# deargen/DeepInteract

Measured on AMD Instinct MI355X. Metric: complexes/sec GeoT+pair-tensor fwd (2×1k res, k=20, 1/8 GPU); % HBM peak, higher is better.
Workload: dtype bf16

## Files before the change

__graft_entry__.py:

```python
import os
import sys

ROOT = os.path.dirname(os.path.abspath(__file__))
if ROOT not in sys.path:
    sys.path.insert(0, ROOT)


def build() -> None:
    from deepinteract_amd import build as _b
    _b.build(force=False)
    import deepinteract_amd
    from deepinteract_amd import _lib
    _lib.load(build_if_missing=False)
    from deepinteract_amd.build import build_variant
    from tools.build_variants import VARIANTS
    for name in ("node2", "f32exact"):
        try:
            build_variant(name, VARIANTS[name])
        except RuntimeError as e:
            print(f"variant {name} failed to build (test_gpu_variants will fail):\n{e}", file=sys.stderr)


def smoke() -> None:
    import numpy as np
    import torch

    from deepinteract_amd.engine import GeoTEngine, PairTensorOp
    from deepinteract_amd.graph import GraphBatch
    from deepinteract_amd.weights import seeded_state_dict
    from oracle import geot_oracle as O

    z = np.load(os.path.join(ROOT, "tests", "golden", "tiny.npz"))
    items, graphs = [], []
    for tag in ("g1", "g2"):
        it = {"num_nodes": int(z[f"{tag}_node_f"].shape[0])}
        for k in ("src", "dst", "src_nbr", "dst_nbr"):
            it[k] = torch.as_tensor(z[f"{tag}_{k}"]).long()
        it["node_f"] = torch.as_tensor(z[f"{tag}_node_f"])
        it["edge_f"] = torch.as_tensor(z[f"{tag}_edge_f"])
        items.append(it)
    sd = seeded_state_dict(0, with_head=False)
    eng = GeoTEngine(sd, "f32", device="cuda:0")
    gb = GraphBatch.from_arrays(items, "cuda:0")
    h, e = eng.forward(gb)
    n1 = items[0]["num_nodes"]
    _, views = PairTensorOp("cuda:0")(h, [0], [n1], [n1], [items[1]["num_nodes"]])
    torch.cuda.synchronize()
    with torch.no_grad():
        ref = [O.geot_forward(sd, it) for it in items]
    ref_h = torch.cat([r[0] for r in ref]).numpy()
    got = h.cpu().numpy()
    err = np.abs(got - ref_h).max() / np.abs(ref_h).max()
    pt_ref = O.pair_tensor(torch.as_tensor(ref_h[:n1]), torch.as_tensor(ref_h[n1:])).numpy()
    perr = np.abs(views[0].cpu().numpy() - pt_ref).max() / np.abs(pt_ref).max()
    print(f"smoke: GeoT node rel err {err:.2e}, pair tensor rel err {perr:.2e}")
    if not (err < 1e-4 and perr < 1e-4):
        raise AssertionError(f"smoke parity failed: {err}, {perr}")


if __name__ == "__main__":
    build()
    if len(sys.argv) > 1 and sys.argv[1] == "smoke":
        smoke()
```

deepinteract_amd/csrc/common.h:

```cpp
#pragma once
#include <hip/hip_runtime.h>
#include <stdint.h>

#include <atomic>

namespace di {

inline int device_cus() {
  constexpr int MAXDEV = 64;
  static std::atomic<int> cache[MAXDEV];
  int dev = 0;
  if (hipGetDevice(&dev) != hipSuccess || dev < 0) dev = 0;
  if (dev < MAXDEV) {
    const int c = cache[dev].load(std::memory_order_relaxed);
    if (c > 0) return c;
  }
  int v = 0;
  if (hipDeviceGetAttribute(&v, hipDeviceAttributeMultiprocessorCount, dev) != hipSuccess || v <= 0) v = 256;
  if (dev < MAXDEV) cache[dev].store(v, std::memory_order_relaxed);
  return v;
}

typedef float floatx4 __attribute__((ext_vector_type(4)));
typedef float floatx2 __attribute__((ext_vector_type(2)));
// ... 287 lines not shown
    const int bo = blk(i), s = kst(i);
    out.v[bo] = __builtin_amdgcn_mfma_f32_16x16x32_bf16(fr[i % D], op.f[s], out.v[bo], 0, 0, 0);
    if (i + D < N)
      fr[i % D] = *reinterpret_cast<const bf16x8*>(w + (blk(i + D) * NS + kst(i + D)) * BLK + lane * 8);
  }
  __builtin_amdgcn_sched_barrier(0);
}

template <int NBO, int NS>
__device__ __forceinline__ void mma(Act<NBO>& out, const Op<BF16T, NS>& op, const u16* w, int lane) {
  constexpr int G = NBO < 2 ? NBO : 2;
#pragma unroll
  for (int b0 = 0; b0 < NBO; b0 += G) {
#pragma unroll
    for (int s = 0; s < NS; ++s) {
#pragma unroll
      for (int bo = b0; bo < b0 + G; ++bo) {
        const bf16x8 af = *reinterpret_cast<const bf16x8*>(w + (bo * NS + s) * BLK + lane * 8);
        out.v[bo] = __builtin_amdgcn_mfma_f32_16x16x32_bf16(af, op.f[s], out.v[bo], 0, 0, 0);
      }
    }
  }
}
template <int NBO, int NS>
__device__ __forceinline__ void mma(Act<NBO>& out, const Op<F32T, NS>& op, const float* w, int lane) {
#pragma unroll
  for (int s = 0; s < NS; ++s)
#pragma unroll
    for (int sub = 0; sub < 2; ++sub) {
#pragma unroll
      for (int bo = 0; bo < NBO; ++bo) {
        const floatx4 a4 = *reinterpret_cast<const floatx4*>(w + (bo * NS + s) * BLK + sub * 256 + lane * 4);
#pragma unroll
        for (int r = 0; r < 4; ++r)
          out.v[bo] = __builtin_amdgcn_mfma_f32_16x16x4f32(a4[r], op.f[2 * s + sub][r], out.v[bo], 0, 0, 0);
      }
      __builtin_amdgcn_sched_barrier(0);
    }
}

template <class DT, int NBO, int NS>
__device__ __forceinline__ void linear(Act<NBO>& out, const Act<2 * NS>& a, const typename DT::T* w, int lane) {
  Op<DT, NS> op;
  make_op(op, a);
  mma<NBO, NS>(out, op, w, lane);
}

__device__ __forceinline__ void lds_dma_wait() { asm volatile("s_waitcnt vmcnt(0)" ::: "memory"); }

template <int NW, typename T>
__device__ __forceinline__ void dma_blocks(T* lds, const T* g, int nblk) {
  const int wave = __builtin_amdgcn_readfirstlane(threadIdx.x >> 6);
  const int loff = (threadIdx.x & 63) * 16;
  const int nkib = nblk * BLK * (int)sizeof(T) / 1024;
  const __amdgpu_buffer_rsrc_t r = buf_rsrc(g);
  for (int i = wave; i < nkib; i += NW)
    __builtin_amdgcn_raw_ptr_buffer_load_lds(
        r, (__attribute__((address_space(3))) void*)(reinterpret_cast<char*>(lds) + i * 1024), 16, loff, i * 1024, 0, 0);
}

template <int NW>
__device__ __forceinline__ void dma_vec(float* lds, const float* g, int n512) {
  const int wave = __builtin_amdgcn_readfirstlane(threadIdx.x >> 6);
  const int lane = threadIdx.x & 63;
  const __amdgpu_buffer_rsrc_t r = buf_rsrc(g);
  if (lane < 32)
    for (int i = wave; i < n512; i += NW)
      __builtin_amdgcn_raw_ptr_buffer_load_lds(
          r, (__attribute__((address_space(3))) void*)(reinterpret_cast<char*>(lds) + i * 512), 16, lane * 16, i * 512, 0, 0);
}

template <typename T, int NW, bool DBUF, int CAP, int VCAP = 0>
struct WPipe {
  static_assert(NW >= 1 && NW <= 16, "waves per block");
  static_assert((CAP * BLK * (int)sizeof(T)) % 1024 == 0, "a stage is whole 1-KiB LDS-DMA pieces");
  static_assert(VCAP % 128 == 0, "bias vectors are whole 512-B pieces");
  static constexpr int SLOT_BYTES = CAP * BLK * (int)sizeof(T) + VCAP * 4;
  char* base;
  int cur;
  const T* pend;
  int pend_n;
  const float* pendv;
  int pendv_n;
  __device__ explicit WPipe(void* lds)
      : base(reinterpret_cast<char*>(lds)), cur(0), pend(nullptr), pend_n(0), pendv(nullptr), pendv_n(0) {}
  __device__ __forceinline__ T* slot_w(int s) const { return reinterpret_cast<T*>(base + (DBUF ? s : 0) * SLOT_BYTES); }
  __device__ __forceinline__ float* slot_v(int s) const {
    return reinterpret_cast<float*>(base + (DBUF ? s : 0) * SLOT_BYTES + CAP * BLK * (int)sizeof(T));
  }
  __device__ __forceinline__ void issue(const T* g, int nblk, const float* gv = nullptr, int nvec = 0) {
    if constexpr (DBUF) {
      dma_blocks<NW>(slot_w(cur ^ 1), g, nblk);
      if (gv) dma_vec<NW>(slot_v(cur ^ 1), gv, nvec / 128);
    } else {
      pend = g;
      pend_n = nblk;
      pendv = gv;
      pendv_n = nvec;
    }
  }
  __device__ __forceinline__ const T* next() {
    if constexpr (DBUF) {
      lds_dma_wait();
      __syncthreads();
      cur ^= 1;
    } else {
      __syncthreads();
      dma_blocks<NW>(slot_w(0), pend, pend_n);
      if (pendv) dma_vec<NW>(slot_v(0), pendv, pendv_n / 128);
      lds_dma_wait();
      __syncthreads();
    }
    return slot_w(cur);
  }
  __device__ __forceinline__ const T* w() const { return slot_w(cur); }
  __device__ __forceinline__ const float* v() const { return slot_v(cur); }
};

template <int NW_>
struct KernelGeo {
  static_assert(NW_ >= 1 && NW_ <= 16, "waves per block");
  static constexpr int NW = NW_;
  static constexpr int THREADS = 64 * NW_;
  static constexpr int ROWS = ROWS_PER_WAVE * NW_;
};

template <typename T>
__device__ __forceinline__ void stage(T* lds, const T* g, int nblk) {
  __syncthreads();
  dma_blocks<WAVES>(lds, g, nblk);
  lds_dma_wait();
  __syncthreads();
}

template <int NB>
__device__ __forceinline__ float head_sum(const Act<NB>& a, int h) {
  float s = 0.f;
#pragma unroll
  for (int r = 0; r < 4; ++r) s += a.v[2 * h][r];
#pragma unroll
  for (int r = 0; r < 4; ++r) s += a.v[2 * h + 1][r];
  s += __shfl_xor(s, 16);
  s += __shfl_xor(s, 32);
  return s;
}

}
```

deepinteract_amd/csrc/geot_edge.hip:

```cpp
#include "geot.h"
#include "mfma32.h"

namespace di {

__constant__ int EL_ORDER[25] = {
    EL_S0, EL_UP, EL_OM,
    EL_RES + 0 * MAT128, EL_RES + 1 * MAT128, EL_RES + 2 * MAT128,
    EL_RES + 3 * MAT128, EL_RES + 4 * MAT128, EL_RES + 5 * MAT128,
    EL_RC,
    EL_RES + 6 * MAT128, EL_RES + 7 * MAT128, EL_RES + 8 * MAT128,
    EL_RES + 9 * MAT128, EL_RES + 10 * MAT128, EL_RES + 11 * MAT128,
    EL_FG, EL_F, EL_P,
    EL_OE, EL_F1, EL_F2, EL_F1 + MAT128, EL_F2 + MAT128, EL_NN};
__constant__ int EL_SIZE[25] = {36, 16, 32, 32, 32, 32, 32, 32, 32, 32, 32, 32, 32,
                                32, 32, 32, 8, 32, 32, 32, 32, 32, 32, 32, 32};
__constant__ int EL_VEC[25] = {-1, ELV_OM, -1,
                               ELV_RES + 0 * 128, ELV_RES + 1 * 128, ELV_RES + 2 * 128,
                               ELV_RES + 3 * 128, ELV_RES + 4 * 128, ELV_RES + 5 * 128,
                               ELV_RC,
                               ELV_RES + 6 * 128, ELV_RES + 7 * 128, ELV_RES + 8 * 128,
                               ELV_RES + 9 * 128, ELV_RES + 10 * 128, ELV_RES + 11 * 128,
                               -1, ELV_F, ELV_P,
                               ELV_OE, ELV_F1, -1, ELV_F1 + 128, -1, ELV_NN};
constexpr int EL_NSTAGE_CONF = 18, EL_NSTAGE_FINAL = 19, EL_NSTAGE = 25;
// ... 271 lines not shown
  });
  pin(x);
}
template <class FB>
__device__ __forceinline__ void x32_f_residual_blk(X32<4>& x, const u16* w, const float* v, FB&& fblk, int lane, int h) {
  P32<8> op;
  make_op32(op, x);
  X32<4> y;
  lin32_pipe<8>(y, op, w, v, lane, h, [&](int b) {
    silu2_blk(y.v[b]);
    const R32<1> fr = fblk(b);
#pragma unroll
    for (int q = 0; q < 4; ++q) set_quad(x.v[b], q, unpack4(fr.u[q]) + silu2_unit<true>() * quad(y.v[b], q));
  });
  pin(x);
}


template <int CTRL, int ROW_MASK>
__device__ __forceinline__ void fold_step(X32<4>& s, floatx4& z, int d) {
  const bool same = __builtin_amdgcn_update_dpp(-2, d, CTRL, ROW_MASK, 0xf, false) == d;
  auto mv = [](float x) {
    return __builtin_bit_cast(float, __builtin_amdgcn_update_dpp(0, __builtin_bit_cast(int, x), CTRL, ROW_MASK, 0xf,
                                                                  false));
  };
#pragma unroll
  for (int b = 0; b < 4; ++b) {
#pragma unroll
    for (int k = 0; k < 16; ++k) {
      const float t = mv(s.v[b][k]);
      s.v[b][k] += same ? t : 0.f;
    }
    const float t = mv(z[b]);
    z[b] += same ? t : 0.f;
  }
}

__device__ __forceinline__ void edge_attn_fold(const EdgeArgs& a, int e, bool valid, int lane, int h, floatx4 al,
                                               int d, const R32<4>& vr, int2 ip) {
  if (!valid) {
    d = -1;
    al = (floatx4){0.f, 0.f, 0.f, 0.f};
  }
  X32<4> s;
#pragma unroll
  for (int b = 0; b < 4; ++b)
#pragma unroll
    for (int q = 0; q < 4; ++q) set_quad(s.v[b], q, al[b] * unpack4(vr.u[4 * b + q]));
  floatx4 z = al;
  fold_step<0x111, 0xf>(s, z, d);
  fold_step<0x112, 0xf>(s, z, d);
  fold_step<0x114, 0xf>(s, z, d);
  fold_step<0x118, 0xf>(s, z, d);
  fold_step<0x142, 0xa>(s, z, d);
  const int dnext = __shfl_down(d, 1, 32);
  if (!valid || ((lane & 31) != 31 && dnext == d)) return;
  const int t = e / FOLD_ROWS, t0 = ip.x / FOLD_ROWS, t1 = (ip.y - 1) / FOLD_ROWS;
  if (t0 == t1) {
    float* row = a.attn_out + (int64_t)d * HID;
#pragma unroll
    for (int b = 0; b < 4; ++b) {
      const float den = z[b] + 1e-6f;
#pragma unroll
      for (int q = 0; q < 4; ++q) {
        const floatx4 x = quad(s.v[b], q);
        st4(row + 32 * b + 8 * q + 4 * h, (floatx4){x[0] / den, x[1] / den, x[2] / den, x[3] / den});
      }
    }
  } else {
    float* p = a.attn_parts + ((int64_t)t * 2 + (t == t0 ? 1 : 0)) * FOLD_PART;
#pragma unroll
    for (int b = 0; b < 4; ++b)
#pragma unroll
      for (int q = 0; q < 4; ++q) st4(p + 32 * b + 8 * q + 4 * h, quad(s.v[b], q));
    if (h == 0) st4(p + HID, z);
  }
}

template <int MODE, bool GC, bool Z0, class ST>
__device__ __forceinline__ void edge_x32_tile(const EdgeArgs& a, ST& st, int e, bool valid, int lane, int h,
                                              const u16* wc2) {
  constexpr bool FINAL = MODE == 1;
  static_assert(!Z0 || (GC && !FINAL), "the z0 form is the non-final DI_GRAPH_GEO_REF layer 0");
  const u16* f_row = reinterpret_cast<const u16*>(a.f_in) + (int64_t)e * HID;
  const u16* qkv = reinterpret_cast<const u16*>(a.qkv);

  P32<2> gop;
  {
    const float* grow = a.edge_f + (int64_t)e * NFEAT_E;
    X32<1> geo;
#pragma unroll
    for (int q = 0; q < 4; ++q) {
      const int f = 8 * q + 4 * h;
      set_quad(geo.v[0], q, f < NFEAT_E ? ld4(grow + f) : (floatx4){0.f, 0.f, 0.f, 0.f});
    }
    make_op32(gop, geo);
  }
  X32<4> x;
  R32<4> fr;
  P32<2> zop;
  auto f0 = [&](int b) { return f0_blk(wc2, zop, b, lane); };
  (void)f0;
  const u16* w;
  if constexpr (Z0) {
    load_z0(zop, reinterpret_cast<const u16*>(a.f_in), e, h);
    w = st.next([&] { asm volatile("" ::"v"(zop.f[0]), "v"(zop.f[1])); });
    init_vec32_lds(x, st.v(), h);
  } else if constexpr (GC) {
    fr.load(f_row, h);
    w = st.next([&] { settle(fr); });
    init_vec32_lds(x, st.v(), h);
  } else {
    const u16* fn_in = reinterpret_cast<const u16*>(a.fn_in);
    const int4 nb = *reinterpret_cast<const int4*>(a.nbr + (int64_t)e * 4);
    R32<4> xn;
    xn.load(fn_in + (int64_t)nb.x * HID, h);
    w = st.next();
    X32<2> gate;
    {
      X32<2> t1;
      zero(gate);
      mma32<2, 2>(gate, gop, w + 8 * BLK, lane);
      zero(t1);
      mma32<2, 2>(t1, gop, w + 12 * BLK, lane);
#pragma unroll
      for (int b = 0; b < 2; ++b) gate.v[b] *= t1.v[b];
      zero(t1);
      mma32<2, 2>(t1, gop, w + 16 * BLK, lane);
#pragma unroll
      for (int b = 0; b < 2; ++b) gate.v[b] *= t1.v[b];
      pin(gate);
    }
    X32<2> s;
    zero(s);
#pragma unroll
    for (int j = 0; j < 4; ++j) {
      P32<8> xop;
#pragma unroll
      for (int b = 0; b < 4; ++b) {
        asm volatile("" ::: "memory");
        floatx16 dg = {};
        dg = mfma32(afrag(w, 2 * b, lane), gop.f[0], dg);
        dg = mfma32(afrag(w, 2 * b + 1, lane), gop.f[1], dg);
#pragma unroll
        for (int t = 0; t < 2; ++t) {
          asm volatile("" : "+v"(xn.u[4 * b + 2 * t]), "+v"(xn.u[4 * b + 2 * t + 1]));
          const floatx4 lo = unpack4(xn.u[4 * b + 2 * t]) * quad(dg, 2 * t);
          const floatx4 hi = unpack4(xn.u[4 * b + 2 * t + 1]) * quad(dg, 2 * t + 1);
          const uint4 u = {pack_bf16x2(lo[0], lo[1]), pack_bf16x2(lo[2], lo[3]), pack_bf16x2(hi[0], hi[1]),
                           pack_bf16x2(hi[2], hi[3])};
          xop.f[2 * b + t] = __builtin_bit_cast(bf16x8, u);
        }
      }
      if (j < 3) {
        const int nx = j == 0 ? nb.y : (j == 1 ? nb.z : nb.w);
        xn.load(fn_in + (int64_t)nx * HID, h);
      }
      X32<2> y;
      zero(y);
      mma32<2, 8>(y, xop, w + 20 * BLK, lane);
#pragma unroll
      for (int b = 0; b < 2; ++b)
#pragma unroll
        for (int k = 0; k < 16; ++k) s.v[b][k] += silu2<true>(y.v[b][k]) * gate.v[b][k];
      pin(s);
    }
    w = st.next();
    {
      P32<4> sop;
      make_op32(sop, s);
      zero(x);
      mma32<4, 4>(x, sop, w, lane);
      X32<4> bo;
      init_vec32_lds(bo, st.v(), h);
#pragma unroll
      for (int b = 0; b < 4; ++b) {
        silu2_blk(x.v[b]);
        x.v[b] = silu2_unit<true>() * x.v[b] + bo.v[b];
      }
      pin(x);
    }
    fr.load(f_row, h);
    w = st.next([&] { settle(fr); });
  }
  {
    P32<8> fop;
    if constexpr (Z0) {
#pragma unroll
      for (int b = 0; b < 4; ++b) {
        lean_fence();
        P32<2> o;
        raw_op32(o, f0(b));
        fop.f[2 * b] = o.f[0];
        fop.f[2 * b + 1] = o.f[1];
        asm volatile("" : "+v"(fop.f[2 * b]), "+v"(fop.f[2 * b + 1]));
      }
    } else {
      raw_op32(fop, fr);
    }
    mma32<4, 8>(x, fop, w, lane);
    pin(x);
  }
  x32_res_block(x, st, lane, h);
  x32_res_block(x, st, lane, h);
  if constexpr (!Z0) fr.load(f_row, h);
  w = st.next([&] { if constexpr (!Z0) settle(fr); });
  if constexpr (Z0) x32_f_residual_blk(x, w, st.v(), f0, lane, h);
  else x32_f_residual(x, w, st.v(), fr, lane, h);
  x32_res_block(x, st, lane, h);
  x32_res_block(x, st, lane, h);
  w = st.next();
  {
    X32<4> fg;
    zero(fg);
    mma32<4, 2>(fg, gop, w, lane);
#pragma unroll
    for (int b = 0; b < 4; ++b) x.v[b] *= fg.v[b];
    pin(x);
  }
  if constexpr (!Z0) fr.load(f_row, h);
  w = st.next([&] { if constexpr (!Z0) settle(fr); });
  if constexpr (Z0) x32_f_residual_blk(x, w, st.v(), f0, lane, h);
  else x32_f_residual(x, w, st.v(), fr, lane, h);

  R32<4> kr, qr;
  const int sn = a.src[e], dn = a.dst[e];
  kr.load(qkv + (int64_t)sn * 3 * HID + HID, h);
  qr.load(qkv + (int64_t)dn * 3 * HID, h);
  const bool fold = !Z0 && a.attn_out != nullptr;
  R32<4> vr;
  int2 ip = {0, 0};
  auto fold_loads = [&] {
    vr.load(qkv + (int64_t)sn * 3 * HID + 2 * HID, h);
    ip = *reinterpret_cast<const int2*>(a.in_ptr + dn);
  };
  if (GC && fold) fold_loads();
  w = st.next([&] {
    settle(kr);
    settle(qr);
    if (GC && fold) {
      settle(vr);
      asm volatile("" ::"v"(ip.x), "v"(ip.y));
    }
  });
  X32<4> p;
  {
    P32<8> xop;
    make_op32(xop, x);
    init_vec32_lds(p, st.v(), h);
    mma32<4, 8>(p, xop, w, lane);
  }
  floatx4 al;
#pragma unroll
  for (int b = 0; b < 4; ++b) {
    float sum = 0.f;
#pragma unroll
    for (int q = 0; q < 4; ++q) {
      const floatx4 kq = unpack4(kr.u[4 * b + q]), qd = unpack4(qr.u[4 * b + q]);
#pragma unroll
      for (int i = 0; i < 4; ++i) {
        float sc = (kq[i] * qd[i]) * (1.0f / 5.656854249492381f);
        sc = fminf(fmaxf(sc, -5.f), 5.f);
        const float pv = sc * p.v[b][4 * q + i];
        p.v[b][4 * q + i] = pv;
        sum += pv;
      }
    }
    sum += __shfl_xor(sum, 32);
    al[b] = expf_<true>(fminf(fmaxf(sum, -5.f), 5.f));
  }
  if (valid && h == 0 && a.alpha_out != nullptr) st4(a.alpha_out + (int64_t)e * 4, al);
  if (!GC && fold) fold_loads();
  if constexpr (FINAL) {
    if (fold) edge_attn_fold(a, e, valid, lane, h, al, dn, vr, ip);
  } else {
    P32<8> pop;
    make_op32(pop, p);
    pin(pop);
    if (fold) edge_attn_fold(a, e, valid, lane, h, al, dn, vr, ip);
    if constexpr (!Z0) fr.load(f_row, h);
    w = st.next([&] { if constexpr (!Z0) settle(fr); });
    X32<4> e1;
    init_vec32_lds(e1, st.v(), h);
    mma32<4, 8>(e1, pop, w, lane);
#pragma unroll
    for (int b = 0; b < 4; ++b) {
      R32<1> fb;
      if constexpr (Z0) {
        lean_fence();
        fb = f0(b);
      } else {
#pragma unroll
        for (int q = 0; q < 4; ++q) fb.u[q] = fr.u[4 * b + q];
      }
#pragma unroll
      for (int q = 0; q < 4; ++q) set_quad(e1.v[b], q, quad(e1.v[b], q) + unpack4(fb.u[q]));
    }
    pin(e1);
    P32<8> eop;
    make_op32(eop, e1);
    pin(eop);
#pragma unroll 1
    for (int half = 0; half < 2; ++half) {
      w = st.next();
      X32<4> t;
      P32<8> top;
      lin32_pipe<8>(t, eop, w, st.v(), lane, h, [&](int b) {
        silu2_blk(t.v[b]);
        pack_blk(top.f[2 * b], top.f[2 * b + 1], t.v[b]);
      });
      pin(top);
      w = st.next();
      mma32<4, 8>(e1, top, w, lane);
      pin(e1);
    }
    if (valid) store_row32(e1, reinterpret_cast<u16*>(a.f_out) + (int64_t)e * HID, h);
    if constexpr (GC) return;
    make_op32(eop, e1);
    w = st.next();
    X32<4> fn;
    init_vec32_lds(fn, st.v(), h);
    mma32<4, 8>(fn, eop, w, lane);
#pragma unroll
    for (int b = 0; b < 4; ++b) silu_blk(fn.v[b]);
    if (valid) store_row32(fn, reinterpret_cast<u16*>(a.fn_out) + (int64_t)e * HID, h);
  }
}

constexpr int RING_NW = 8, RING_SLOTS = 4, RING_AHEAD = 2;
using RingSlot = WPipe<u16, RING_NW, true, EL_CAP, 128>;
struct EdgeRingGeo {
  static constexpr int NW = RING_NW, THREADS = 64 * NW, ROWS_PER_WAVE = 32, ROWS = ROWS_PER_WAVE * NW;
};
static_assert(EdgeRingGeo::ROWS_PER_WAVE == FOLD_ROWS, "a fold tile is one wave's rows");

__device__ __forceinline__ uint32_t lds_off(const uint32_t* p) {
  return (uint32_t)(uintptr_t)(const __attribute__((address_space(3))) uint32_t*)p;
}
__device__ __forceinline__ uint32_t lds_ld(const uint32_t* p) {
  uint32_t v;
  asm volatile("ds_read_b32 %0, %1\n\ts_waitcnt lgkmcnt(0)" : "=v"(v) : "v"(lds_off(p)) : "memory");
  return v;
}
__device__ __forceinline__ void lds_add(uint32_t* p) {
  asm volatile(
      "s_mov_b64 s[0:1], exec\n\t"
      "s_mov_b64 exec, 1\n\t"
      "ds_add_u32 %0, %1\n\t"
      "s_mov_b64 exec, s[0:1]" ::"v"(lds_off(p)), "v"(1u)
      : "memory", "s0", "s1");
}
__device__ __forceinline__ void lds_wait_ge(const uint32_t* p, uint32_t v) {
  while (lds_ld(p) < v) __builtin_amdgcn_s_sleep(1);
}

typedef uint32_t rsrc4 __attribute__((ext_vector_type(4)));
__device__ __forceinline__ rsrc4 rsrc_of(const void* p) {
  const uint64_t a = (uint64_t)(uintptr_t)p;
  return (rsrc4){(uint32_t)__builtin_amdgcn_readfirstlane((int)(uint32_t)a),
                 (uint32_t)__builtin_amdgcn_readfirstlane((int)(uint32_t)(a >> 32)) & 0xffffu, 0x7fffffffu,
                 (uint32_t)BUF_RSRC_W3};
}
__device__ __forceinline__ void dma_piece(rsrc4 r, uint32_t lds, int voff, int soff) {
  asm volatile(
      "s_mov_b32 m0, %0\n\t"
      "s_nop 0\n\t"
      "buffer_load_dwordx4 %1, %2, %3 offen lds" ::"s"(__builtin_amdgcn_readfirstlane((int)lds)),
      "v"(voff), "s"(r), "s"(__builtin_amdgcn_readfirstlane(soff))
      : "memory", "m0");
}

struct RingPieces {
  const u16* w;
  int off[3], n[3];
  int np;
  const float* v;
};
template <int NS, bool GC>
struct EdgeRingSrc {
  const u16* W;
  const float* V;
  __device__ RingPieces operator()(int gs) const {
    const int s = gs % NS;
    const int si = GC ? s + 2 : s;
    const int vo = (GC && s == 0) ? ELV_OM : EL_VEC[si];
    return {W, {EL_ORDER[si], 0, 0}, {EL_SIZE[si], 0, 0}, 1, vo >= 0 ? V + vo : nullptr};
  }
};

template <class SRC, int NW = RING_NW>
struct RingStagesT {
  char* base;
  uint32_t* full;
  uint32_t* freec;
  SRC src;
  int wave;
  int total;
  int g = 0;
  int issued = 0;
  int pending = -1;
  int cur = 0;
  __device__ u16* slot_w(int sl) const { return reinterpret_cast<u16*>(base + sl * RingSlot::SLOT_BYTES); }
  __device__ float* slot_v(int sl) const {
    return reinterpret_cast<float*>(base + sl * RingSlot::SLOT_BYTES + EL_CAP * BLK * 2);
  }
  __device__ void issue_one(int gs) {
    const RingPieces p = src(gs);
    const int sl = gs % RING_SLOTS;
// ... 176 lines not shown
```

deepinteract_amd/csrc/geot_init.hip:

```cpp
#include "geot.h"
#include "mfma32.h"
#include "pair_queue.h"

namespace di {

using EmbedGeo = KernelGeo<4>;
template <class DT>
__global__ __launch_bounds__(EmbedGeo::THREADS) void k_node_embed(EmbedArgs a) {
  pq_signal_at_start(a.sig_q, a.sig_job);
  using T = typename DT::T;
  __shared__ __attribute__((aligned(16))) T lds[2 * MAT128 * BLK];
  const int lane = lane_id(), g = lane >> 4;
  const int r = row_id<EmbedGeo::NW>();
  const bool valid = r < a.Nt;
  const int v = valid ? r : a.Nt - 1;
  const T* W = reinterpret_cast<const T*>(a.wmat);
  WPipe<T, EmbedGeo::NW, true, MAT128> pipe(lds);
  pipe.issue(W + EM_EMB * BLK, MAT128);

  Act<8> x;
  const float* row = a.node_f + (int64_t)v * a.in_dim;
#pragma unroll
  for (int b = 0; b < 8; ++b)
#pragma unroll
// ... 217 lines not shown
        if (t > 0) silu2_blk(y);
        gs += y;
      }
      acc.v[b] *= gs;
      asm volatile("" : "+v"(acc.v[b]));
    }
  }
  const u16* w = wt(2 + NT);
  P32<8> aop;
  make_op32(aop, acc);
  X32<1> z;
  zero(z);
  mma32<1, 8>(z, aop, w, lane);
  make_op32(zop, z);
  return w;
}
template <bool GC, class WT, class GO>
__device__ __forceinline__ void init_tile_x32(X32<4>& acc, const P32<2>& gop, const float* wvec, int lane, int h,
                                              WT&& wt, GO&& gate_off, X32<4>& f) {
  P32<2> zop;
  const u16* w = init_tile_x32_z<GC>(acc, gop, wvec, lane, h, wt, gate_off, zop);
  zero(f);
  mma32<4, 2>(f, zop, w + 8 * BLK, lane);
}

__device__ __forceinline__ void init_acc_x32(X32<4>& acc, const InitArgs& a, int ps, int pd, int h) {
  const float* rs = a.pos_src + (int64_t)ps * HID;
  const float* rd = a.pos_dst + (int64_t)pd * HID;
#pragma unroll
  for (int b = 0; b < 4; ++b)
#pragma unroll
    for (int q = 0; q < 4; ++q) {
      const int f = 32 * b + 8 * q + 4 * h;
      set_quad(acc.v[b], q, ld4(rs + f) + ld4(rd + f));
    }
}

template <bool ONE = false>
__device__ __forceinline__ void geo_op32(P32<2>& gop, const float* edge_f, int e, int h) {
  const float* grow = edge_f + (int64_t)e * NFEAT_E;
  X32<1> geo;
#pragma unroll
  for (int q = 0; q < 4; ++q) {
    const int f = 8 * q + 4 * h;
    set_quad(geo.v[0], q, f < NFEAT_E ? ld4(grow + f) : (ONE ? (floatx4){1.f, 1.f, 0.f, 0.f} : (floatx4){0.f, 0.f, 0.f, 0.f}));
  }
  make_op32(gop, geo);
}

template <bool GC, bool Z = false>
__global__ __attribute__((amdgpu_flat_work_group_size(1, InitX32Geo::THREADS), amdgpu_waves_per_eu(3, 3),
                          amdgpu_num_vgpr(80)))
void k_init_x32(InitArgs a, EmbedArgs ea, int embed_blocks) {
  static_assert(GC || !Z, "the z0 form is the DI_GRAPH_GEO_REF path");
  pq_signal_at_start(ea.sig_q, ea.sig_job);
  using G = InitGeo<BF16T>;
  constexpr int NW = InitX32Geo::NW;
  __shared__ __attribute__((aligned(16))) u16 lds[G::CAP * BLK];
  const int lane = lane_id();
  if ((int)blockIdx.x < embed_blocks) {
    WPipe<u16, NW, false, G::CAP> epipe(lds);
    embed_block<BF16T, NW>(ea, epipe, blockIdx.x, lane, lane >> 4);
    return;
  }
  const int h = lane >> 5;
  const int r = ((int)blockIdx.x - embed_blocks) * InitX32Geo::ROWS + (threadIdx.x >> 6) * InitX32Geo::ROWS_PER_WAVE +
                (lane & 31);
  const bool valid = r < a.Et;
  const int e = valid ? r : a.Et - 1;
  const u16* W = reinterpret_cast<const u16*>(a.wmat);
  WPipe<u16, NW, false, G::CAP> pipe(lds);
  pipe.issue(W + IE_T0 * BLK, 8);
  P32<2> gop;
  geo_op32<GC>(gop, a.edge_f, e, h);
  X32<4> acc;
  init_acc_x32(acc, a, a.node_pos[a.src[e]], a.node_pos[a.dst[e]], h);
  const bool with_fn = a.fn_out != nullptr;
  constexpr int NT = GC ? 2 : 4;
  auto geo_t = [](int i) { return GC ? (i == 0 ? 1 : 4) : i + 1; };
  auto wt = [&](int p) -> const u16* {
    const u16* w = pipe.next();
    if (p == 0) pipe.issue(W + (IE_T0 + 40 * geo_t(0)) * BLK, 40);
    else if (p < NT) pipe.issue(W + (IE_T0 + 40 * geo_t(p)) * BLK, 40);
    else if (p == NT) pipe.issue(W + IE_GEO1 * BLK, 40);
    else if (p == NT + 1) pipe.issue(W + IE_C1 * BLK, Z ? 8 : 16);
    else if (with_fn) pipe.issue(W + IE_NBR * BLK, MAT128);
    return w;
  };
  if constexpr (Z) {
    P32<2> zop;
    init_tile_x32_z<GC>(acc, gop, a.wvec, lane, h, wt, [](int t) { return 8 * t; }, zop);
    if (valid) store_z0(zop, reinterpret_cast<u16*>(a.f_out), e, h);
    return;
  }
  X32<4> f;
  init_tile_x32<GC>(acc, gop, a.wvec, lane, h, wt, [](int t) { return 8 * t; }, f);
  if (valid) store_row32(f, reinterpret_cast<u16*>(a.f_out) + (int64_t)e * HID, h);
  if (!with_fn) return;
  const u16* w = pipe.next();
  P32<8> fop;
  make_op32(fop, f);
  X32<4> fn;
  init_vec32(fn, a.wvec + IEV_NBR, h);
  mma32<4, 8>(fn, fop, w, lane);
#pragma unroll
  for (int b = 0; b < 4; ++b) silu_blk(fn.v[b]);
  if (valid) store_row32(fn, reinterpret_cast<u16*>(a.fn_out) + (int64_t)e * HID, h);
}

constexpr int IRX_NW = 12;
__global__ __attribute__((amdgpu_flat_work_group_size(1, 64 * IRX_NW), amdgpu_waves_per_eu(IRX_NW / 4, IRX_NW / 4)))
void k_init_res_x32(InitArgs a, int ntiles) {
  __shared__ __attribute__((aligned(16))) u16 w[IR_NBLK * BLK];
  const u16* W = reinterpret_cast<const u16*>(a.wmat);
  dma_blocks<IRX_NW>(w + IR_T0 * BLK, W + IE_T0 * BLK, 8);
  dma_blocks<IRX_NW>(w + IR_DIST * BLK, W + (IE_T0 + 40 * 1) * BLK, 40);
  dma_blocks<IRX_NW>(w + IR_AMIDE * BLK, W + (IE_T0 + 40 * 4) * BLK, 40);
  dma_blocks<IRX_NW>(w + IR_GATE * BLK, W + IE_GEO1 * BLK, 16);
  dma_blocks<IRX_NW>(w + (IR_GATE + 16) * BLK, W + (IE_GEO1 + 32) * BLK, 8);
  dma_blocks<IRX_NW>(w + IR_C * BLK, W + IE_C1 * BLK, 16);
  lds_dma_wait();
  __syncthreads();
  const int lane = lane_id(), h = lane >> 5;
  const int wave = __builtin_amdgcn_readfirstlane(threadIdx.x >> 6);
  const int stride = gridDim.x * IRX_NW;
  auto edge_of = [&](int t) {
    const int r = t * 32 + (lane & 31);
    return r < a.Et ? r : a.Et - 1;
  };
  int tile = blockIdx.x * IRX_NW + wave;
  int ps = 0, pd = 0;
  if (tile < ntiles) {
    const int e = edge_of(tile);
    ps = a.node_pos[a.src[e]];
    pd = a.node_pos[a.dst[e]];
  }
  auto wt = [&](int p) -> const u16* {
    return w + (p == 0 ? IR_T0 : p == 1 ? IR_DIST : p == 2 ? IR_AMIDE : p == 3 ? IR_GATE : IR_C) * BLK;
  };
  auto gate_off = [](int t) { return t == 0 ? 0 : (t == 1 ? 8 : 16); };
#pragma unroll 1
  for (; tile < ntiles; tile += stride) {
    const int r = tile * 32 + (lane & 31);
    const bool valid = r < a.Et;
    const int e = valid ? r : a.Et - 1;
    P32<2> gop;
    geo_op32<true>(gop, a.edge_f, e, h);
    X32<4> acc;
    init_acc_x32(acc, a, ps, pd, h);
    const bool more = tile + stride < ntiles;
    if (more) {
      const int en = edge_of(tile + stride);
      ps = a.node_pos[a.src[en]];
      pd = a.node_pos[a.dst[en]];
    }
    X32<4> f;
    init_tile_x32<true>(acc, gop, a.wvec, lane, h, wt, gate_off, f);
    if (valid) store_row32(f, reinterpret_cast<u16*>(a.f_out) + (int64_t)e * HID, h);
  }
}

}

using namespace di;

extern "C" int di_node_embed(const di_graph* g, di_dtype dt, int32_t in_dim, const float* node_f, const void* wmat,
                             const float* wvec, void* h_out, void* qkv_out, void* queue, int32_t signal_job,
                             void* stream) {
  if (!g || !node_f || !wmat || !wvec || !h_out || !qkv_out || g->num_nodes <= 0 || in_dim <= 0 || in_dim > HID ||
      !dtype_ok(dt))
    return DI_EINVAL;
  EmbedArgs a{g->num_nodes, in_dim, node_f, wmat, wvec, h_out, qkv_out, (uint32_t*)queue, signal_job};
  hipStream_t s = (hipStream_t)stream;
  if (dt == DI_BF16)
    hipLaunchKernelGGL(k_node_embed<BF16T>, grid_of<EmbedGeo>(a.Nt), block_of<EmbedGeo>(), 0, s, a);
  else
    hipLaunchKernelGGL(k_node_embed<F32T>, grid_of<EmbedGeo>(a.Nt), block_of<EmbedGeo>(), 0, s, a);
  return launch_status();
}

extern "C" int di_init_edge(const di_graph* g, di_dtype dt, const float* edge_f, const void* wmat,
                            const float* wvec, const float* pos_src_tab, const float* pos_dst_tab,
                            void* f_out, void* fn_out, void* stream) {
  const bool gc = (g ? g->flags : 0) & DI_GRAPH_GEO_REF;
  if (!g || !edge_f || !wmat || !wvec || !pos_src_tab || !pos_dst_tab || !f_out || (!fn_out && !gc) ||
      g->num_edges <= 0 || !dtype_ok(dt))
    return DI_EINVAL;
  InitArgs a{g->num_edges, edge_f, g->src, g->dst, g->node_pos, wmat, wvec, pos_src_tab, pos_dst_tab,
             f_out, fn_out};
  hipStream_t s = (hipStream_t)stream;
  const dim3 gf = grid_of<InitGeo<F32T>>(a.Et), bf = block_of<InitGeo<F32T>>();
  const EmbedArgs ne{};
  const dim3 gx((unsigned)((a.Et + InitX32Geo::ROWS - 1) / InitX32Geo::ROWS)), bx(InitX32Geo::THREADS);
  if (dt == DI_BF16 && gc) hipLaunchKernelGGL((k_init_x32<true>), gx, bx, 0, s, a, ne, 0);
  else if (dt == DI_BF16) hipLaunchKernelGGL((k_init_x32<false>), gx, bx, 0, s, a, ne, 0);
  else if (gc) hipLaunchKernelGGL((k_init_edge<F32T, true>), gf, bf, 0, s, a, ne, 0);
  else hipLaunchKernelGGL((k_init_edge<F32T, false>), gf, bf, 0, s, a, ne, 0);
  return launch_status();
}

template <class DT, bool Z = false>
static void launch_embed_init(const InitArgs& a, const EmbedArgs& ea, hipStream_t s) {
  if constexpr (DT::kBF16) {
    const int eb = (ea.Nt + InitX32Geo::EMBED_ROWS - 1) / InitX32Geo::EMBED_ROWS;
    const int ib = (a.Et + InitX32Geo::ROWS - 1) / InitX32Geo::ROWS;
    hipLaunchKernelGGL((k_init_x32<true, Z>), dim3((unsigned)(eb + ib)), dim3(InitX32Geo::THREADS), 0, s, a, ea, eb);
  } else {
    using G = InitGeo<DT>;
    const int eb = (ea.Nt + G::ROWS - 1) / G::ROWS;
    const int ib = (a.Et + G::ROWS - 1) / G::ROWS;
    hipLaunchKernelGGL((k_init_edge<DT, true>), dim3((unsigned)(eb + ib)), block_of<G>(), 0, s, a, ea, eb);
  }
}

static int embed_init_edge(bool z, const di_graph* g, di_dtype dt, int32_t in_dim, const float* node_f,
                           const void* embed_wmat, const float* embed_wvec, void* h_out, void* qkv_out,
                           const float* edge_f, const void* init_wmat, const float* init_wvec,
                           const float* pos_src_tab, const float* pos_dst_tab, void* out, void* queue,
                           int32_t signal_job, void* stream) {
  if (!g || !(g->flags & DI_GRAPH_GEO_REF) || !g->src || !g->dst || !g->node_pos || g->num_nodes <= 0 ||
      g->num_edges <= 0 || in_dim <= 0 || in_dim > HID || !node_f || !embed_wmat || !embed_wvec || !h_out ||
      !qkv_out || !edge_f || !init_wmat || !init_wvec || !pos_src_tab || !pos_dst_tab || !out ||
      (z ? dt != DI_BF16 : !dtype_ok(dt)))
    return DI_EINVAL;
  EmbedArgs ea{g->num_nodes, in_dim, node_f, embed_wmat, embed_wvec, h_out, qkv_out, (uint32_t*)queue, signal_job};
  InitArgs a{g->num_edges, edge_f, g->src, g->dst, g->node_pos, init_wmat, init_wvec, pos_src_tab, pos_dst_tab,
             out, nullptr};
  hipStream_t s = (hipStream_t)stream;
  if (z) launch_embed_init<BF16T, true>(a, ea, s);
  else if (dt == DI_BF16) launch_embed_init<BF16T>(a, ea, s);
  else launch_embed_init<F32T>(a, ea, s);
  return launch_status();
}

extern "C" int di_embed_init_edge(const di_graph* g, di_dtype dt, int32_t in_dim, const float* node_f,
                                  const void* embed_wmat, const float* embed_wvec, void* h_out, void* qkv_out,
                                  const float* edge_f, const void* init_wmat, const float* init_wvec,
                                  const float* pos_src_tab, const float* pos_dst_tab, void* f_out, void* queue,
                                  int32_t signal_job, void* stream) {
  return embed_init_edge(false, g, dt, in_dim, node_f, embed_wmat, embed_wvec, h_out, qkv_out, edge_f, init_wmat,
                         init_wvec, pos_src_tab, pos_dst_tab, f_out, queue, signal_job, stream);
// ... 23 lines not shown
```

deepinteract_amd/csrc/mfma32.h:

```cpp
#pragma once
#include "common.h"

namespace di {

typedef float floatx16 __attribute__((ext_vector_type(16)));

template <int NB>
struct X32 {
  floatx16 v[NB];
};
template <int NS>
struct P32 {
  bf16x8 f[NS];
};
template <int NB>
struct R32 {
  uint2 u[4 * NB];
  __device__ __forceinline__ void load(const u16* row, int h) {
#pragma unroll
    for (int b = 0; b < NB; ++b)
#pragma unroll
      for (int q = 0; q < 4; ++q) u[4 * b + q] = *reinterpret_cast<const uint2*>(row + 32 * b + 8 * q + 4 * h);
  }
};

constexpr int Z0_ROW = 32;
__device__ __forceinline__ void load_z0(P32<2>& z, const u16* zbuf, int64_t e, int h) {
  const u16* p = zbuf + e * Z0_ROW + 16 * h;
  z.f[0] = *reinterpret_cast<const bf16x8*>(p);
  z.f[1] = *reinterpret_cast<const bf16x8*>(p + 8);
}
__device__ __forceinline__ void store_z0(const P32<2>& z, u16* zbuf, int64_t e, int h) {
  u16* p = zbuf + e * Z0_ROW + 16 * h;
  *reinterpret_cast<bf16x8*>(p) = z.f[0];
  *reinterpret_cast<bf16x8*>(p + 8) = z.f[1];
}

__device__ __forceinline__ floatx4 unpack4(uint2 u) {
  return (floatx4){__builtin_bit_cast(float, u.x << 16), __builtin_bit_cast(float, u.x & 0xffff0000u),
                   __builtin_bit_cast(float, u.y << 16), __builtin_bit_cast(float, u.y & 0xffff0000u)};
}
__device__ __forceinline__ floatx4 quad(const floatx16& v, int q) {
  return (floatx4){v[4 * q], v[4 * q + 1], v[4 * q + 2], v[4 * q + 3]};
}
__device__ __forceinline__ void set_quad(floatx16& v, int q, floatx4 x) {
  v[4 * q] = x[0];
  v[4 * q + 1] = x[1];
  v[4 * q + 2] = x[2];
  v[4 * q + 3] = x[3];
}

template <int NB>
__device__ __forceinline__ void zero(X32<NB>& a) {
#pragma unroll
  for (int b = 0; b < NB; ++b) a.v[b] = (floatx16){};
}
template <int NB>
__device__ __forceinline__ void init_vec32_lds(X32<NB>& a, const float* vec, int h) {
  const __attribute__((address_space(3))) floatx4* p = (const __attribute__((address_space(3))) floatx4*)vec;
#pragma unroll
  for (int b = 0; b < NB; ++b)
#pragma unroll
    for (int q = 0; q < 4; ++q) set_quad(a.v[b], q, p[8 * b + 2 * q + h]);
}
template <int NB>
__device__ __forceinline__ void init_vec32(X32<NB>& a, const float* vec, int h) {
#pragma unroll
  for (int b = 0; b < NB; ++b)
#pragma unroll
    for (int q = 0; q < 4; ++q) set_quad(a.v[b], q, ld4(vec + 32 * b + 8 * q + 4 * h));
}
template <int NB>
__device__ __forceinline__ void to_x32(X32<NB>& a, const R32<NB>& r) {
#pragma unroll
  for (int b = 0; b < NB; ++b)
#pragma unroll
    for (int q = 0; q < 4; ++q) set_quad(a.v[b], q, unpack4(r.u[4 * b + q]));
}
template <int NB>
__device__ __forceinline__ void store_row32(const X32<NB>& a, u16* row, int h) {
#pragma unroll
  for (int b = 0; b < NB; ++b)
#pragma unroll
    for (int q = 0; q < 4; ++q) {
      const floatx4 x = quad(a.v[b], q);
      *reinterpret_cast<uint2*>(row + 32 * b + 8 * q + 4 * h) = (uint2){pack_bf16x2(x[0], x[1]), pack_bf16x2(x[2], x[3])};
    }
}

__device__ __forceinline__ void pack_blk(bf16x8& f0, bf16x8& f1, const floatx16& v) {
  uint4 u0, u1;
  u0.x = pack_bf16x2(v[0], v[1]);
  u0.y = pack_bf16x2(v[2], v[3]);
  u0.z = pack_bf16x2(v[4], v[5]);
  u0.w = pack_bf16x2(v[6], v[7]);
  u1.x = pack_bf16x2(v[8], v[9]);
  u1.y = pack_bf16x2(v[10], v[11]);
  u1.z = pack_bf16x2(v[12], v[13]);
  u1.w = pack_bf16x2(v[14], v[15]);
  f0 = __builtin_bit_cast(bf16x8, u0);
  f1 = __builtin_bit_cast(bf16x8, u1);
}
template <int NB>
__device__ __forceinline__ void make_op32(P32<2 * NB>& o, const X32<NB>& a) {
#pragma unroll
  for (int b = 0; b < NB; ++b) pack_blk(o.f[2 * b], o.f[2 * b + 1], a.v[b]);
}
template <int NB>
__device__ __forceinline__ void raw_op32(P32<2 * NB>& o, const R32<NB>& r) {
#pragma unroll
  for (int b = 0; b < NB; ++b)
#pragma unroll
    for (int t = 0; t < 2; ++t) {
      const uint2 lo = r.u[4 * b + 2 * t], hi = r.u[4 * b + 2 * t + 1];
      o.f[2 * b + t] = __builtin_bit_cast(bf16x8, (uint4){lo.x, lo.y, hi.x, hi.y});
    }
}

template <int NB>
__device__ __forceinline__ void pin(X32<NB>& a) {
#pragma unroll
  for (int b = 0; b < NB; ++b) asm volatile("" : "+v"(a.v[b]));
}
template <int NS>
__device__ __forceinline__ void pin(P32<NS>& o) {
#pragma unroll
  for (int s = 0; s < NS; ++s) asm volatile("" : "+v"(o.f[s]));
}
template <int NB>
__device__ __forceinline__ void settle(const R32<NB>& r) {
#pragma unroll
  for (int i = 0; i < 4 * NB; ++i) asm volatile("" ::"v"(r.u[i].x), "v"(r.u[i].y));
}

__device__ __forceinline__ void silu2_blk(floatx16& v) {
#pragma unroll
  for (int k = 0; k < 16; ++k) v[k] = silu2<true>(v[k]);
}
__device__ __forceinline__ void silu_blk(floatx16& v) {
#pragma unroll
  for (int k = 0; k < 16; ++k) v[k] = silu<true>(v[k]);
}

__device__ __forceinline__ floatx16 mfma32(const bf16x8& a, const bf16x8& b, const floatx16& c) {
  return __builtin_amdgcn_mfma_f32_32x32x16_bf16(a, b, c, 0, 0, 0);
}
__device__ __forceinline__ bf16x8 afrag(const u16* w, int blk, int lane) {
  return *reinterpret_cast<const bf16x8*>(w + blk * BLK + lane * 8);
}

__device__ __forceinline__ R32<1> f0_blk(const u16* wc2, const P32<2>& z, int b, int lane) {
  floatx16 fb = {};
  fb = mfma32(afrag(wc2, 2 * b, lane), z.f[0], fb);
  fb = mfma32(afrag(wc2, 2 * b + 1, lane), z.f[1], fb);
  R32<1> r;
#pragma unroll
  for (int q = 0; q < 4; ++q) {
    const floatx4 x = quad(fb, q);
    r.u[q] = (uint2){pack_bf16x2(x[0], x[1]), pack_bf16x2(x[2], x[3])};
  }
  return r;
}

template <int NBO, int NS>
__device__ __forceinline__ void mma32(X32<NBO>& out, const P32<NS>& op, const u16* w, int lane) {
  constexpr int N = NBO * NS;
  constexpr int D = MMA_DEPTH < N ? MMA_DEPTH : N;
  bf16x8 fr[D];
#pragma unroll
  for (int i = 0; i < D; ++i) fr[i] = afrag(w, i, lane);
#pragma unroll
  for (int i = 0; i < N; ++i) {
    __builtin_amdgcn_sched_barrier(0);
    out.v[i / NS] = mfma32(fr[i % D], op.f[i % NS], out.v[i / NS]);
    if (i + D < N) fr[i % D] = afrag(w, i + D, lane);
  }
  __builtin_amdgcn_sched_barrier(0);
}

constexpr int PIPE32_NV = 8;
constexpr int PIPE32_LEAD = 1;
template <int NS, class Epi>
__device__ __forceinline__ void lin32_pipe(X32<4>& out, const P32<NS>& op, const u16* w, const float* bias, int lane,
                                           int h, Epi&& epi) {
  constexpr int NBO = 4, N = NBO * NS, D = MMA_DEPTH < N ? MMA_DEPTH : N;
  if (bias) init_vec32_lds(out, bias, h);
  else zero(out);
  bf16x8 fr[D];
#pragma unroll
  for (int i = 0; i < D; ++i) fr[i] = afrag(w, i, lane);
  __builtin_amdgcn_sched_barrier(0);
#pragma unroll
  for (int ob = 0; ob < NBO; ++ob) {
#pragma unroll
    for (int s = 0; s < NS; ++s) {
      const int i = ob * NS + s;
      out.v[ob] = mfma32(fr[i % D], op.f[s], out.v[ob]);
      if (i + D < N) fr[i % D] = afrag(w, i + D, lane);
    }
    if (ob > 0) epi(ob - 1);
    __builtin_amdgcn_sched_group_barrier(0x008, PIPE32_LEAD, 0);
#pragma unroll
    for (int s = PIPE32_LEAD; s < NS + PIPE32_LEAD; ++s) {
      __builtin_amdgcn_sched_group_barrier(0x402, PIPE32_NV, 0);
      __builtin_amdgcn_sched_group_barrier(0x100, 1, 0);
      if (s < NS) __builtin_amdgcn_sched_group_barrier(0x008, 1, 0);
    }
    __builtin_amdgcn_sched_barrier(0);
  }
  epi(NBO - 1);
}

}
```

Measured before the change: 8659.

## Widen edge-row loads/stores to 16-byte vectors with permlane32 swaps

Row loads and stores of 128-wide bf16 edge features now use 16-byte vector accesses per lane instead of 8-byte ones. Lanes exchange halves with permlane32_swap to map between the wide memory layout and the MFMA 32x32 register layout. The aim is fewer, wider global memory transactions on this bandwidth-bound edge pipeline. The change also makes stores predicated inside the helper, trims the gated-conv geo weight DMA to only the blocks used via a second pending transfer, and registers a rows8 build variant. The extra cross-lane swaps add VALU work and register pressure.

```diff
diff --git a/__graft_entry__.py b/__graft_entry__.py
--- a/__graft_entry__.py
+++ b/__graft_entry__.py
@@ -14,11 +14,11 @@
     _lib.load(build_if_missing=False)
     from deepinteract_amd.build import build_variant
     from tools.build_variants import VARIANTS
-    for name in ("node2", "f32exact"):
+    for name in ("node2", "f32exact", "rows8"):
         try:
             build_variant(name, VARIANTS[name])
         except RuntimeError as e:
-            print(f"variant {name} failed to build (test_gpu_variants will fail):\n{e}", file=sys.stderr)
+            print(f"variant {name} failed to build (its GPU test will fail):\n{e}", file=sys.stderr)
 
 
 def smoke() -> None:
diff --git a/deepinteract_amd/csrc/common.h b/deepinteract_amd/csrc/common.h
--- a/deepinteract_amd/csrc/common.h
+++ b/deepinteract_amd/csrc/common.h
@@ -393,8 +393,11 @@
   int pend_n;
   const float* pendv;
   int pendv_n;
+  const T* pend2;
+  int pend2_n;
   __device__ explicit WPipe(void* lds)
-      : base(reinterpret_cast<char*>(lds)), cur(0), pend(nullptr), pend_n(0), pendv(nullptr), pendv_n(0) {}
+      : base(reinterpret_cast<char*>(lds)), cur(0), pend(nullptr), pend_n(0), pendv(nullptr), pendv_n(0),
+        pend2(nullptr), pend2_n(0) {}
   __device__ __forceinline__ T* slot_w(int s) const { return reinterpret_cast<T*>(base + (DBUF ? s : 0) * SLOT_BYTES); }
   __device__ __forceinline__ float* slot_v(int s) const {
     return reinterpret_cast<float*>(base + (DBUF ? s : 0) * SLOT_BYTES + CAP * BLK * (int)sizeof(T));
@@ -408,7 +411,14 @@
       pend_n = nblk;
       pendv = gv;
       pendv_n = nvec;
+      pend2 = nullptr;
+      pend2_n = 0;
     }
+  }
+  __device__ __forceinline__ void issue2(const T* g2, int n2) {
+    static_assert(!DBUF, "issue2 is the single-slot pipe's");
+    pend2 = g2;
+    pend2_n = n2;
   }
   __device__ __forceinline__ const T* next() {
     if constexpr (DBUF) {
@@ -418,6 +428,7 @@
     } else {
       __syncthreads();
       dma_blocks<NW>(slot_w(0), pend, pend_n);
+      if (pend2_n > 0) dma_blocks<NW>(slot_w(0) + pend_n * BLK, pend2, pend2_n);
       if (pendv) dma_vec<NW>(slot_v(0), pendv, pendv_n / 128);
       lds_dma_wait();
       __syncthreads();
diff --git a/deepinteract_amd/csrc/geot_edge.hip b/deepinteract_amd/csrc/geot_edge.hip
--- a/deepinteract_amd/csrc/geot_edge.hip
+++ b/deepinteract_amd/csrc/geot_edge.hip
@@ -377,6 +377,7 @@
                                               const u16* wc2) {
   constexpr bool FINAL = MODE == 1;
   static_assert(!Z0 || (GC && !FINAL), "the z0 form is the non-final DI_GRAPH_GEO_REF layer 0");
+  asm volatile("" : "+v"(h));
   const u16* f_row = reinterpret_cast<const u16*>(a.f_in) + (int64_t)e * HID;
   const u16* qkv = reinterpret_cast<const u16*>(a.qkv);
 
@@ -434,6 +435,7 @@
 #pragma unroll
       for (int b = 0; b < 4; ++b) {
         asm volatile("" ::: "memory");
+        xn.unswz_blk(b);
         floatx16 dg = {};
         dg = mfma32(afrag(w, 2 * b, lane), gop.f[0], dg);
         dg = mfma32(afrag(w, 2 * b + 1, lane), gop.f[1], dg);
@@ -566,13 +568,17 @@
   }
   if (valid && h == 0 && a.alpha_out != nullptr) st4(a.alpha_out + (int64_t)e * 4, al);
   if (!GC && fold) fold_loads();
+  auto attn_fold = [&] {
+    if (!GC) vr.unswz();
+    edge_attn_fold(a, e, valid, lane, h, al, dn, vr, ip);
+  };
   if constexpr (FINAL) {
-    if (fold) edge_attn_fold(a, e, valid, lane, h, al, dn, vr, ip);
+    if (fold) attn_fold();
   } else {
     P32<8> pop;
     make_op32(pop, p);
     pin(pop);
-    if (fold) edge_attn_fold(a, e, valid, lane, h, al, dn, vr, ip);
+    if (fold) attn_fold();
     if constexpr (!Z0) fr.load(f_row, h);
     w = st.next([&] { if constexpr (!Z0) settle(fr); });
     X32<4> e1;
@@ -609,7 +615,7 @@
       mma32<4, 8>(e1, top, w, lane);
       pin(e1);
     }
-    if (valid) store_row32(e1, reinterpret_cast<u16*>(a.f_out) + (int64_t)e * HID, h);
+    store_row32(e1, reinterpret_cast<u16*>(a.f_out) + (int64_t)e * HID, h, valid);
     if constexpr (GC) return;
     make_op32(eop, e1);
     w = st.next();
@@ -618,7 +624,7 @@
     mma32<4, 8>(fn, eop, w, lane);
 #pragma unroll
     for (int b = 0; b < 4; ++b) silu_blk(fn.v[b]);
-    if (valid) store_row32(fn, reinterpret_cast<u16*>(a.fn_out) + (int64_t)e * HID, h);
+    store_row32(fn, reinterpret_cast<u16*>(a.fn_out) + (int64_t)e * HID, h, valid);
   }
 }
 
diff --git a/deepinteract_amd/csrc/geot_init.hip b/deepinteract_amd/csrc/geot_init.hip
--- a/deepinteract_amd/csrc/geot_init.hip
+++ b/deepinteract_amd/csrc/geot_init.hip
@@ -323,20 +323,35 @@
     const u16* w = pipe.next();
     if (p == 0) pipe.issue(W + (IE_T0 + 40 * geo_t(0)) * BLK, 40);
     else if (p < NT) pipe.issue(W + (IE_T0 + 40 * geo_t(p)) * BLK, 40);
-    else if (p == NT) pipe.issue(W + IE_GEO1 * BLK, 40);
+    else if (p == NT) {
+      if constexpr (GC) {
+        pipe.issue(W + IE_GEO1 * BLK, 16);
+        pipe.issue2(W + (IE_GEO1 + 32) * BLK, 8);
+      } else {
+        pipe.issue(W + IE_GEO1 * BLK, 40);
+      }
+    }
     else if (p == NT + 1) pipe.issue(W + IE_C1 * BLK, Z ? 8 : 16);
     else if (with_fn) pipe.issue(W + IE_NBR * BLK, MAT128);
     return w;
   };
+  auto gate_off = [](int t) { return GC ? (t == 0 ? 0 : (t == 1 ? 8 : 16)) : 8 * t; };
   if constexpr (Z) {
     P32<2> zop;
-    init_tile_x32_z<GC>(acc, gop, a.wvec, lane, h, wt, [](int t) { return 8 * t; }, zop);
+    init_tile_x32_z<GC>(acc, gop, a.wvec, lane, h, wt, gate_off, zop);
     if (valid) store_z0(zop, reinterpret_cast<u16*>(a.f_out), e, h);
     return;
   }
+  auto store_f = [&](const X32<4>& t, void* out) {
+    int l = __builtin_amdgcn_mbcnt_hi(~0u, __builtin_amdgcn_mbcnt_lo(~0u, 0u));
+    asm volatile("" : "+v"(l));
+    const int rr = ((int)blockIdx.x - embed_blocks) * InitX32Geo::ROWS + (threadIdx.x >> 6) * InitX32Geo::ROWS_PER_WAVE +
+                   (l & 31);
+    store_row32(t, reinterpret_cast<u16*>(out) + (int64_t)e * HID, l >> 5, rr < a.Et);
+  };
   X32<4> f;
-  init_tile_x32<GC>(acc, gop, a.wvec, lane, h, wt, [](int t) { return 8 * t; }, f);
-  if (valid) store_row32(f, reinterpret_cast<u16*>(a.f_out) + (int64_t)e * HID, h);
+  init_tile_x32<GC>(acc, gop, a.wvec, lane, h, wt, gate_off, f);
+  store_f(f, a.f_out);
   if (!with_fn) return;
   const u16* w = pipe.next();
   P32<8> fop;
@@ -346,7 +361,7 @@
   mma32<4, 8>(fn, fop, w, lane);
 #pragma unroll
   for (int b = 0; b < 4; ++b) silu_blk(fn.v[b]);
-  if (valid) store_row32(fn, reinterpret_cast<u16*>(a.fn_out) + (int64_t)e * HID, h);
+  store_f(fn, a.fn_out);
 }
 
 constexpr int IRX_NW = 12;
@@ -397,7 +412,7 @@
     }
     X32<4> f;
     init_tile_x32<true>(acc, gop, a.wvec, lane, h, wt, gate_off, f);
-    if (valid) store_row32(f, reinterpret_cast<u16*>(a.f_out) + (int64_t)e * HID, h);
+    store_row32(f, reinterpret_cast<u16*>(a.f_out) + (int64_t)e * HID, h, valid);
   }
 }
 
diff --git a/deepinteract_amd/csrc/mfma32.h b/deepinteract_amd/csrc/mfma32.h
--- a/deepinteract_amd/csrc/mfma32.h
+++ b/deepinteract_amd/csrc/mfma32.h
@@ -13,14 +13,48 @@
 struct P32 {
   bf16x8 f[NS];
 };
+#ifndef DI_ROW_WIDE
+#define DI_ROW_WIDE 1
+#endif
+
+typedef uint32_t row16 __attribute__((ext_vector_type(4), aligned(8)));
+
+__device__ __forceinline__ void swap32(uint32_t& a, uint32_t& b) {
+  const auto r = __builtin_amdgcn_permlane32_swap(a, b, false, false);
+  a = r[0];
+  b = r[1];
+}
+
 template <int NB>
 struct R32 {
   uint2 u[4 * NB];
   __device__ __forceinline__ void load(const u16* row, int h) {
+#if DI_ROW_WIDE
+#pragma unroll
+    for (int j = 0; j < 2 * NB; ++j) {
+      const row16 w = *reinterpret_cast<const row16*>(row + 16 * j + 8 * h);
+      u[2 * j] = (uint2){w[0], w[1]};
+      u[2 * j + 1] = (uint2){w[2], w[3]};
+    }
+#else
 #pragma unroll
     for (int b = 0; b < NB; ++b)
 #pragma unroll
       for (int q = 0; q < 4; ++q) u[4 * b + q] = *reinterpret_cast<const uint2*>(row + 32 * b + 8 * q + 4 * h);
+#endif
+  }
+  __device__ __forceinline__ void unswz_blk(int b) {
+#if DI_ROW_WIDE
+#pragma unroll
+    for (int t = 0; t < 2; ++t) {
+      swap32(u[4 * b + 2 * t].x, u[4 * b + 2 * t + 1].x);
+      swap32(u[4 * b + 2 * t].y, u[4 * b + 2 * t + 1].y);
+    }
+#endif
+  }
+  __device__ __forceinline__ void unswz() {
+#pragma unroll
+    for (int b = 0; b < NB; ++b) unswz_blk(b);
   }
 };
 
@@ -78,14 +112,28 @@
     for (int q = 0; q < 4; ++q) set_quad(a.v[b], q, unpack4(r.u[4 * b + q]));
 }
 template <int NB>
-__device__ __forceinline__ void store_row32(const X32<NB>& a, u16* row, int h) {
+__device__ __forceinline__ void store_row32(const X32<NB>& a, u16* row, int h, bool valid) {
+#if DI_ROW_WIDE
+#pragma unroll
+  for (int j = 0; j < 2 * NB; ++j) {
+    const floatx4 x = quad(a.v[j / 2], 2 * (j % 2)), y = quad(a.v[j / 2], 2 * (j % 2) + 1);
+    uint32_t x0 = pack_bf16x2(x[0], x[1]), x1 = pack_bf16x2(x[2], x[3]);
+    uint32_t y0 = pack_bf16x2(y[0], y[1]), y1 = pack_bf16x2(y[2], y[3]);
+    swap32(x0, y0);
+    swap32(x1, y1);
+    if (valid) *reinterpret_cast<row16*>(row + 16 * j + 8 * h) = (row16){x0, x1, y0, y1};
+    __builtin_amdgcn_sched_barrier(0);
+  }
+#else
 #pragma unroll
   for (int b = 0; b < NB; ++b)
 #pragma unroll
     for (int q = 0; q < 4; ++q) {
       const floatx4 x = quad(a.v[b], q);
-      *reinterpret_cast<uint2*>(row + 32 * b + 8 * q + 4 * h) = (uint2){pack_bf16x2(x[0], x[1]), pack_bf16x2(x[2], x[3])};
-    }
+      if (valid)
+        *reinterpret_cast<uint2*>(row + 32 * b + 8 * q + 4 * h) = (uint2){pack_bf16x2(x[0], x[1]), pack_bf16x2(x[2], x[3])};
+    }
+#endif
 }
 
 __device__ __forceinline__ void pack_blk(bf16x8& f0, bf16x8& f1, const floatx16& v) {
@@ -128,9 +176,10 @@
   for (int s = 0; s < NS; ++s) asm volatile("" : "+v"(o.f[s]));
 }
 template <int NB>
-__device__ __forceinline__ void settle(const R32<NB>& r) {
+__device__ __forceinline__ void settle(R32<NB>& r) {
 #pragma unroll
   for (int i = 0; i < 4 * NB; ++i) asm volatile("" ::"v"(r.u[i].x), "v"(r.u[i].y));
+  r.unswz();
 }
 
 __device__ __forceinline__ void silu2_blk(floatx16& v) {
```

Measured after the change: 8905 (median of 6 runs). +2.8%, better.
